# vision-agh/apse_uav

Measured on AMD Instinct MI355X. Metric: 4K UAV frames/sec (whole node), higher is better.
Workload: dtype f32

## Files before the change

### apse_uav_amd/_lib.py

```python
import ctypes as C
import os

import numpy as np

_HERE = os.path.dirname(os.path.abspath(__file__))
_TREE_LIB = os.path.join(_HERE, "libapse_hip.so")
LIB_PATH = os.environ.get("APSE_HIP_LIB") or _TREE_LIB
TOOL_ENTRIES = ("apse_conv2d_ex", "apse_winograd_pack_filter", "apse_winograd_conv2d", "apse_winograd_conv2d_split", "apse_conv_pointwise_launches", "apse_lane_stats", "apse_rpn_select", "apse_box_inference",
                "apse_c4_rpn_select", "apse_rpn_select_train", "apse_rpn_train_proposals_workspace_bytes", "apse_rpn_train_proposals",
                "apse_set_rpn_head", "apse_roi_features_windows", "apse_set_crop_features", "apse_preprocess_frames_yuv", "apse_yuv_to_bgr", "apse_yuv_matrix_host", "apse_resize_normalize_yuv")

APSE_OK = 0


class ApseError(RuntimeError):
    pass


class Config(C.Structure):
    _fields_ = [
        ("struct_size", C.c_int), ("device", C.c_int), ("max_batch", C.c_int),
        ("frame_h", C.c_int), ("frame_w", C.c_int), ("image_h", C.c_int), ("image_w", C.c_int),
        ("blocks", C.c_int * 4), ("num_classes", C.c_int),
        ("score_thresh", C.c_float), ("box_nms", C.c_float), ("rpn_nms", C.c_float), ("mask_thresh", C.c_float),
        ("rpn_pre_topk", C.c_int), ("rpn_post_topk", C.c_int), ("dets_per_image", C.c_int),
        ("pixel_mean", C.c_float * 3), ("assoc_roi", C.c_int), ("embed_dim", C.c_int), ("assoc_scale", C.c_float),
        ("compute_dtype", C.c_int), ("storage16", C.c_int),
    ]


class ConfigArch(Config):
    _fields_ = [("arch", C.c_int)]


class ConfigLane(ConfigArch):
    _fields_ = [("tail_lane", C.c_int)]


class ResultsLayout(C.Structure):
    _fields_ = [("bytes", C.c_size_t), ("n_max", C.c_int), ("dets_per_image", C.c_int), ("embed_dim", C.c_int),
                ("max_batch", C.c_int)] + [(k, C.c_size_t) for k in (
                    "total", "offset", "prop_count", "img", "cls", "roi", "score", "box_resized", "box", "valid", "rect",
                    "mass", "centroid", "closest", "embedding")]


class RenderItem(C.Structure):
    _fields_ = [("image", C.c_int), ("rect", C.c_int * 4), ("words_per_row", C.c_int), ("bits", C.c_void_p),
                ("box", C.c_float * 4), ("rgb", C.c_uint8 * 4), ("label_off", C.c_int), ("label_len", C.c_int)]


class MotsWindow(C.Structure):
    _fields_ = [("rect", C.c_int * 4), ("words_per_row", C.c_int), ("area", C.c_int), ("bits", C.c_void_p)]


class MotsObject(C.Structure):
    _fields_ = [("rect", C.c_int * 4), ("words_per_row", C.c_int), ("score", C.c_float), ("bits", C.c_void_p)]


class ConvDesc(C.Structure):
    _fields_ = [(k, C.c_int) for k in ("B", "H", "W", "Cin", "Cout", "KH", "KW", "stride", "pad", "relu", "res_mode",
                                       "cfg", "splitk", "prec", "fuse_reduce", "x_st", "res_st", "y_st")]


vp, i, f, sz = C.c_void_p, C.c_int, C.c_float, C.c_size_t
SIGNATURES = {
    "apse_create": ([C.POINTER(Config), C.POINTER(vp)], i),
    "apse_destroy": ([vp], None),
    "apse_last_error": ([vp], C.c_char_p),
    "apse_version": ([], C.c_char_p),
    "apse_set_weight": ([vp, C.c_char_p, vp, C.POINTER(C.c_int64), i], i),
    "apse_finalize_weights": ([vp], i),
    "apse_set_resize_tables": ([vp, vp, vp, i, vp, vp, i], i),
    "apse_set_camera": ([vp, C.POINTER(C.c_double), C.POINTER(C.c_double), i, vp, i, i], i),
    "apse_preprocess_frames": ([vp, vp, i, vp], i),
    "apse_preprocess_images": ([vp, vp, i, vp], i),
    "apse_backbone": ([vp, i, vp], i),
    "apse_rpn": ([vp, i, vp], i),
    "apse_rpn_levels": ([vp, i, i, vp], i),
    "apse_box_head": ([vp, i, vp], i),
    "apse_set_detections": ([vp, vp, vp, vp, vp, i, vp], i),
    "apse_mask_tail": ([vp, i, vp], i),
    "apse_embed": ([vp, i, vp], i),
    "apse_forward": ([vp, i, vp], i),
    "apse_results_describe": ([vp, C.POINTER(ResultsLayout)], i),
    "apse_read_results": ([vp, vp, sz, vp], i),
    "apse_read_results_begin": ([vp, vp, sz, vp], i),
    "apse_read_results_end": ([vp, vp], i),
    "apse_lane_stats": ([vp, C.POINTER(C.c_longlong * 4)], i),
    "apse_copy_mask_window": ([vp, i, i, i, i, i, vp, vp], i),
    "apse_copy_mask_windows": ([vp, i, vp, vp, vp, vp, vp], i),
    "apse_host_copy": ([vp, vp, sz, i], i),
    "apse_feature_shape": ([vp, C.c_char_p, C.POINTER(C.c_int * 3)], i),
    "apse_export_feature": ([vp, C.c_char_p, vp, i, vp], i),
    "apse_debug_tensor": ([vp, C.c_char_p, vp, sz, C.POINTER(sz), vp], i),
    "apse_flops": ([vp, i, C.c_double, C.c_double], C.c_double),
    "apse_profile": ([vp, i], i),
    "apse_profile_read": ([vp, C.POINTER(C.c_double * 42), i], i),
    "apse_conv_packed_elems": ([C.POINTER(ConvDesc)], sz),
    "apse_conv_pack_weight": ([C.POINTER(ConvDesc), vp, i, vp, vp], i),
    "apse_conv2d": ([C.POINTER(ConvDesc), vp, vp, vp, vp, vp, vp, sz, vp], i),
    "apse_conv2d_ex": ([C.POINTER(ConvDesc), vp, vp, vp, vp, vp, vp, sz, vp, i, i, i, vp], i),
    "apse_winograd_pack_filter": ([vp, i, i, vp], i),
    "apse_winograd_conv2d": ([C.POINTER(ConvDesc), vp, vp, vp, vp, vp], i),
    "apse_winograd_conv2d_split": ([C.POINTER(ConvDesc), vp, vp, vp, vp, vp, C.c_size_t, i, vp], i),
    "apse_conv_pointwise_launches": ([], C.c_uint),
    "apse_maxpool3x3s2": ([vp, vp, i, i, i, i, vp], i),
    "apse_maxpool3x3s2_typed": ([vp, vp, i, i, i, i, i, vp], i),
    "apse_roi_align": ([C.POINTER(vp), C.POINTER(i), C.POINTER(i), vp, i, i, i, vp, vp], i),
    "apse_roi_align_typed": ([C.POINTER(vp), C.POINTER(i), C.POINTER(i), vp, i, i, i, i, vp, vp], i),
    "apse_roi_pool": ([vp, i, i, vp, vp, i, i, f, vp, vp], i),
    "apse_roi_features": ([vp, i, vp, vp, i, i, vp, vp], i),
    "apse_roi_features_windows": ([vp, i, vp, vp, i, i, vp, vp], i),
    "apse_set_crop_features": ([vp, i], i),
    "apse_nms_rank": ([vp, vp, vp, i, i, i, i, f, i, vp, vp, vp, vp, vp], i),
    "apse_rpn_select": ([C.POINTER(vp), C.POINTER(i), C.POINTER(i), i, i, i, i, i, i, f, i, vp, vp, vp, vp, vp, vp, vp, vp, vp], i),
    "apse_box_inference": ([vp, i, i, vp, vp, i, i, i, i, f, f, i, i] + [vp] * 16, i),
    "apse_c4_rpn_select": ([vp, i, i, i, i, i, i, i, f, vp, vp, vp, vp, vp, vp, vp, vp], i),
    "apse_mask_centroid_dense": ([vp, i, i, C.POINTER(C.c_int * 3), vp], i),
    "apse_mask_closest_dense": ([vp, i, i, f, f, C.POINTER(C.c_int * 2), vp], i),
    "apse_l2_normalize": ([vp, vp, i, i, vp], i),
    "apse_sqdist": ([vp, vp, i, i, i, vp, vp], i),
    "apse_undistort_gamma": ([vp, vp, i, i, i, C.POINTER(C.c_double), C.POINTER(C.c_double), i, vp, i, i, vp], i),
    "apse_lab_tables_host": ([vp, vp, C.c_size_t], C.c_size_t),
    "apse_replay_create": ([i, i, f, i], vp),
    "apse_replay_destroy": ([vp], None),
    "apse_replay_step": ([vp, i, i, vp, vp, vp, C.c_char_p, i, vp], i),
    "apse_replay_packed": ([vp, vp, C.c_longlong, i, i, i, vp, C.c_longlong], C.c_longlong),
    "apse_replay_max_id": ([vp], i),
    "apse_replay_next_id": ([vp], i),
    "apse_render_workspace_bytes": ([i, i, i], sz),
    "apse_render_instances": ([vp, vp, i, i, i, i, vp, i, vp, sz, vp, i, vp, sz, vp], i),
    "apse_render_pack_mask": ([vp, i, i, vp, vp], i),
    "apse_render_font_host": ([vp, sz], sz),
    "apse_mots_split_workspace_bytes": ([], sz),
    "apse_mots_split_idmap": ([vp, i, i, i, vp, sz, vp, vp, vp, vp, sz, vp], i),
    "apse_mots_rle_to_bits": ([vp, vp, i, i, i, vp, vp], i),
    "apse_mots_overlaps": ([vp, i, vp, i, vp, i, vp, vp], i),
    "apse_mots_shift_overlaps": ([vp, i, vp, i, i, i, vp, vp], i),
    "apse_mots_render_idmap": ([vp, vp, i, i, i, vp, vp], i),
    "apse_mots_crop_overlaps": ([vp, vp, i, i, i, vp, sz, vp, vp, vp], i),
    "apse_mots_rle_workspace_bytes": ([vp, i, i, i], sz),
    "apse_mots_bits_to_rle": ([vp, vp, i, i, i, vp, i, vp, vp, vp, sz, vp], i),
    "apse_mots_rle_pack_workspace_bytes": ([i], sz),
    "apse_mots_rle_pack": ([vp, vp, i, i, vp, i, vp, vp, vp, sz, vp], i),
    "apse_resize_normalize": ([vp, vp, vp, vp, vp, vp, i, vp, vp, i, i, i, i, i, i, i, i, C.POINTER(f * 3), vp], i),
    "apse_assoc_fc_workspace_bytes": ([i, i, i], sz),
    "apse_assoc_fc_forward": ([vp, vp, vp, i, i, i, vp, vp, vp, sz, vp], i),
    "apse_assoc_fc_backward": ([vp, vp, vp, vp, i, i, i, vp, vp, vp, sz, vp], i),
    "apse_triplet_workspace_bytes": ([i], sz),
    "apse_triplet_hard_forward": ([vp, vp, i, i, f, i, vp, vp, sz, vp], i),
    "apse_triplet_all_forward": ([vp, vp, i, i, f, i, vp, vp, sz, vp], i),
    "apse_triplet_hard_backward": ([vp, i, i, i, vp, vp, vp, vp], i),
    "apse_triplet_all_backward": ([vp, i, i, i, vp, vp, vp, vp], i),
    "apse_sgd_step": ([vp, vp, vp, C.c_longlong, f, f, f, f, i, i, vp], i),
    "apse_coco_box_iou": ([vp, vp, vp, i, i, i, vp, vp, vp, vp, vp], i),
    "apse_coco_poly_to_bits": ([vp, vp, i, vp, i, vp, vp, vp, i, vp, vp, vp, vp], i),
    "apse_coco_match": ([vp, vp, vp, i, i, i, vp, vp, vp, i, vp, vp, vp, i, vp, i, vp, i, vp, vp, vp, vp, vp], i),
    "apse_coco_accumulate_workspace_bytes": ([C.c_longlong], sz),
# ... 90 lines not shown
```

### apse_uav_amd/csrc/conv_igemm.hip

```cpp
#include "apse_common.h"
#include <atomic>
#include <type_traits>

typedef _Float16 f16x8 __attribute__((ext_vector_type(8)));
__device__ __forceinline__ f32x16 apse_mfma16(bf16x8 a, bf16x8 b, f32x16 c) { return __builtin_amdgcn_mfma_f32_32x32x16_bf16(a, b, c, 0, 0, 0); }
__device__ __forceinline__ f32x16 apse_mfma16(f16x8 a, f16x8 b, f32x16 c) { return __builtin_amdgcn_mfma_f32_32x32x16_f16(a, b, c, 0, 0, 0); }

struct apse_pointwise {};
template <int WM, int WN, int TM, int TN, int KS, int XT, int WK, int PR = 0, typename... FORM>
__global__ __launch_bounds__(64 * WM * WN * WK) void conv_igemm_f32(const ConvParams p) {
    static_assert(sizeof...(FORM) == 0 || (sizeof...(FORM) == 1 && (std::is_same<FORM, apse_pointwise>::value && ...)), "FORM is nothing or apse_pointwise");
    constexpr bool PW = sizeof...(FORM) != 0;
    static_assert(PR == 0 || XT == 0, "16-bit operands use the descriptor path only");
    static_assert(!PW || XT == 0, "the pointwise address form exists for the plain descriptor path only");
    constexpr bool DESC = XT != 1;
    constexpr int EPS = PR ? 64 : 32;
    constexpr int ESH = PR ? 1 : 2;
    constexpr int EPSLOT = 16 >> ESH;
    constexpr int NT = 64 * WM * WN * WK;
    constexpr int BM = WM * TM * 32;
    constexpr int BN = WN * TN * 32;
    constexpr int SR = NT / 8;
    constexpr int AP = BM / SR;
    constexpr int BP = BN / SR;
    static_assert(AP >= 1 && BP >= 1 && KS % WK == 0 && (DESC || WK == 1), "unsupported shape");
    constexpr int LDC = BN + 4;
    constexpr bool DP = DESC && (TM * TN <= 2 || (PR != 0 && WM * WN == 8 && APSE_DP16));
    constexpr int NSET = DP ? 2 : 1;
    constexpr int STORE_AT = 4 * KS - 2;
    extern __shared__ __attribute__((aligned(16))) char smem[];
    float* As = reinterpret_cast<float*>(smem);
    float* Bs = As + 2 * KS * BM * 32;
    float* Cs = reinterpret_cast<float*>(smem);

    const int tid = threadIdx.x;
    const int lane = tid & 63;
    const int wave = tid >> 6;
    const int kg = wave / (WM * WN);
    const int wm = (wave % (WM * WN)) / WN, wn = wave % WN;
    const int fr = lane & 31, fh = lane >> 5;
    const int srow = tid >> 3, slot = tid & 7;

    int M = p.M;
    if (p.m_count) {
        int lim = (*p.m_count) * p.m_per_item;
        M = lim < M ? lim : M;
    }
    const int tiles_n = (p.Cout + BN - 1) / BN;
    const int tiles_m = (M + BM - 1) / BM;
    const int nwg = tiles_m * tiles_n;
    const int z = blockIdx.y;
    const int steps_per_row = p.KWCp / EPS;
    const int steps_total = PR ? p.KH * steps_per_row : p.steps_total;
    const int steps_big = (steps_total + KS - 1) / KS;
    const int per = (steps_big + p.splitk - 1) / p.splitk;
    const int s_begin = z * per;
    const int s_end = (s_begin + per < steps_big) ? s_begin + per : steps_big;
    const int ohw = p.OH * p.OW;
    const size_t w_row = (size_t)p.KH * p.KWCp;
    const bool direct = (p.splitk == 1);
    __amdgpu_buffer_rsrc_t xrsrc;
    const unsigned xbytes = (((unsigned)(p.B * p.H * p.W) << p.cin_log2)) << (XT >= 2 ? 1 : ESH);
    if constexpr (DESC)
        xrsrc = __builtin_amdgcn_make_buffer_rsrc(const_cast<float*>(p.x), 0, (int)xbytes, 0x00020000);
    __amdgpu_buffer_rsrc_t wrsrc;
    if constexpr (PW)
        wrsrc = __builtin_amdgcn_make_buffer_rsrc(PR ? const_cast<void*>(reinterpret_cast<const void*>(p.w16)) : const_cast<void*>(reinterpret_cast<const void*>(p.w)), 0,
                                                  (int)(((unsigned)((p.Cout + 127) & ~127) * (unsigned)w_row) << ESH), 0x00020000);

    bool warm_pending = p.next_w && z == 0;
    for (int wg = blockIdx.x; wg < nwg; wg += gridDim.x) {
        const int bid = apse_xcd_remap(wg, nwg);
        const int tile_m = bid / tiles_n, tile_n = bid - tile_m * tiles_n;
        const int m0 = tile_m * BM, n0 = tile_n * BN;

        int a_iy0[AP], a_ix0[AP], a_pix[AP], a_base[AP];
#pragma unroll
        for (int i = 0; i < AP; ++i) {
            const int m = m0 + srow + SR * i;
            if (m < M) {
                const int b = m / ohw;
                const int rem = m - b * ohw;
                const int oy = rem / p.OW;
                const int ox = rem - oy * p.OW;
                a_iy0[i] = oy * p.stride - p.pad;
                a_ix0[i] = ox * p.stride - p.pad;
                a_pix[i] = b * p.H * p.W;
            } else {
                a_iy0[i] = -(1 << 28);
                a_ix0[i] = 0;
                a_pix[i] = 0;
            }
            a_base[i] = (a_pix[i] + a_iy0[i] * p.W + a_ix0[i]) << p.cin_log2;
        }

        f32x4 ra[NSET][KS][AP], rb[NSET][KS][BP];
        int ld_r, ld_q;
        {
            const int ss0 = s_begin * KS;
            ld_r = ss0 / steps_per_row;
            ld_q = ss0 - ld_r * steps_per_row;
        }
        const char* wrow[BP];
#pragma unroll
        for (int i = 0; i < BP; ++i)
            wrow[i] = (PR ? reinterpret_cast<const char*>(p.w16) : reinterpret_cast<const char*>(p.w)) +
                      ((((size_t)(n0 + srow + SR * i) * w_row) + (size_t)(slot * EPSLOT)) << ESH);
        int cur_r = 0, cur_ry = 0, cur_q = 0, cur_rowoff = 0, cur_woff = 0, cur_dpx = 0;
        unsigned pw_a[AP], pw_w[BP];
        int pw_s = s_begin * KS, pw_soff = 0;
        unsigned pw_xbytes = 0;
        if constexpr (PW) {
#pragma unroll
            for (int i = 0; i < AP; ++i) {
                const bool in = ((unsigned)a_iy0[i] < (unsigned)p.H) & ((unsigned)a_ix0[i] < (unsigned)p.W);
                pw_a[i] = in ? ((unsigned)(a_base[i] + slot * EPSLOT) << ESH) : 0xfffffff0u;
            }
#pragma unroll
            for (int i = 0; i < BP; ++i) pw_w[i] = ((unsigned)(n0 + srow + SR * i) * (unsigned)w_row + (unsigned)(slot * EPSLOT)) << ESH;
        }
        auto fetch_piece = [&](int set, int u, int j) {
            if constexpr (PW) {
                if (j == 0) {
                    const bool live = pw_s < steps_total;
                    pw_soff = live ? pw_s * 128 : 0;
                    pw_xbytes = live ? xbytes : 0u;
                    ++pw_s;
                }
                if (j < AP) {
                    const __amdgpu_buffer_rsrc_t xs = __builtin_amdgcn_make_buffer_rsrc(const_cast<float*>(p.x), 0, (int)pw_xbytes, 0x00020000);
                    ra[set][u][j] = __builtin_bit_cast(f32x4, __builtin_amdgcn_raw_buffer_load_b128(xs, (int)pw_a[j], pw_soff, 0));
                } else {
                    rb[set][u][j - AP] = __builtin_bit_cast(f32x4, __builtin_amdgcn_raw_buffer_load_b128(wrsrc, (int)pw_w[j - AP], pw_soff, 0));
                }
                return;
            }
            if (j == 0) {
                const bool live = ld_r < p.KH;
                cur_r = live ? ld_r : p.KH - 1;
                cur_ry = live ? ld_r : (1 << 28);
                cur_q = ld_q * EPS + slot * EPSLOT;
                cur_dpx = cur_q >> p.cin_log2;
                cur_rowoff = ((cur_r * p.W) << p.cin_log2) + cur_q;
                cur_woff = (cur_r * p.KWCp + ld_q * EPS) << ESH;
                ++ld_q;
                if (ld_q == steps_per_row) { ld_q = 0; ++ld_r; }
            }
            if (j < AP) {
                const int iy = a_iy0[j] + cur_ry;
                const int px = a_ix0[j] + cur_dpx;
                const int okm = -(int)(((unsigned)iy < (unsigned)p.H) & ((unsigned)px < (unsigned)p.W));
                if constexpr (XT >= 2) {
                    const unsigned off = (((unsigned)(a_base[j] + cur_rowoff) << 1) & (unsigned)okm) | (0xfffffff0u & ~(unsigned)okm);
                    const auto raw = __builtin_amdgcn_raw_buffer_load_b64(xrsrc, (int)off, 0, 0);
                    ra[set][u][j] = f32x4{__uint_as_float(raw[0]), __uint_as_float(raw[1]), 0.f, 0.f};
                } else {
                    const unsigned off = (((unsigned)(a_base[j] + cur_rowoff) << ESH) & (unsigned)okm) | (0xfffffff0u & ~(unsigned)okm);
                    ra[set][u][j] = __builtin_bit_cast(f32x4, __builtin_amdgcn_raw_buffer_load_b128(xrsrc, (int)off, 0, 0));
                }
            } else {
                rb[set][u][j - AP] = *reinterpret_cast<const f32x4*>(wrow[j - AP] + cur_woff);
            }
        };
        auto store_piece = [&](int set, int buf, int u, int j) {
            if (j < AP) {
                const int row = srow + SR * j;
                const int ps = slot ^ ((row >> 1) & 7);
                f32x4 v = ra[set][u][j];
                if constexpr (XT == 2) {
                    const unsigned lo = __float_as_uint(v[0]), hi = __float_as_uint(v[1]);
                    v = f32x4{__uint_as_float(lo << 16), __uint_as_float(lo & 0xffff0000u), __uint_as_float(hi << 16), __uint_as_float(hi & 0xffff0000u)};
                } else if constexpr (XT == 3) {
                    typedef _Float16 h2 __attribute__((ext_vector_type(2)));
                    const h2 a = __builtin_bit_cast(h2, __float_as_uint(v[0])), b = __builtin_bit_cast(h2, __float_as_uint(v[1]));
                    v = f32x4{(float)a[0], (float)a[1], (float)b[0], (float)b[1]};
                }
                *reinterpret_cast<f32x4*>(As + (buf * KS + u) * BM * 32 + row * 32 + ps * 4) = v;
            } else {
                const int row = srow + SR * (j - AP);
                const int ps = slot ^ ((row >> 1) & 7);
                *reinterpret_cast<f32x4*>(Bs + (buf * KS + u) * BN * 32 + row * 32 + ps * 4) = rb[set][u][j - AP];
            }
        };
        auto load_step_bl = [&](int set) {
#pragma unroll
            for (int u = 0; u < KS; ++u)
// ... 437 lines not shown
__global__ __launch_bounds__(256) void conv_splitk_reduce(const ConvParams p) {
    int M = p.M;
    if (p.m_count) {
        int lim = (*p.m_count) * p.m_per_item;
        M = lim < M ? lim : M;
    }
    const size_t total = (size_t)M * p.Cout;
    const int ohw = p.OH * p.OW;
    for (size_t e = (size_t)blockIdx.x * blockDim.x + threadIdx.x; e < total; e += (size_t)gridDim.x * blockDim.x) {
        const int m = (int)(e / p.Cout);
        const int n = (int)(e - (size_t)m * p.Cout);
        float val = 0.f;
        for (int z = 0; z < p.splitk; ++z) val += p.ws[((size_t)z * p.M + m) * p.Cout + n];
        int co = n, g = 0;
        if (p.out_mode == 1) { g = n / p.cdec; co = n - g * p.cdec; }
        if (p.bias) val += p.bias[co];
        auto ld1 = [&](size_t idx) -> float {
            if (p.res_st == 0) return p.res[idx];
            if (p.res_st == 1) return __uint_as_float((uint32_t)reinterpret_cast<const uint16_t*>(p.res)[idx] << 16);
            return (float)reinterpret_cast<const _Float16*>(p.res)[idx];
        };
        size_t dst;
        if (p.out_mode == 0) {
            if (p.res_mode == 1) {
                val += ld1((size_t)m * p.Cout + n);
            } else if (p.res_mode == 2) {
                const int b = m / ohw;
                const int rem = m - b * ohw;
                const int oy = rem / p.OW, ox = rem - oy * p.OW;
                const int hw2 = (p.OH >> 1) * (p.OW >> 1);
                val += ld1(((size_t)b * hw2 + (oy >> 1) * (p.OW >> 1) + (ox >> 1)) * p.Cout + n);
            }
            dst = (size_t)m * p.y_ld + p.y_coff + n;
        } else {
            const int b = m / ohw;
            const int rem = m - b * ohw;
            const int oy = rem / p.OW, ox = rem - oy * p.OW;
            const int dy = g >> 1, dx = g & 1;
            dst = (((size_t)b * 2 * p.OH + 2 * oy + dy) * (2 * p.OW) + 2 * ox + dx) * p.cdec + co;
        }
        if (p.relu) val = apse_relu(val);
        apse_st1(p.y, dst, val, p.y_st);
    }
}

void apse_launch_splitk_reduce4(const ConvParams& p, hipStream_t s) {
    int blocks = (int)(((size_t)p.M * p.Cout / 4 + 255) / 256);
    if (blocks > 4096) blocks = 4096;
    hipLaunchKernelGGL(conv_splitk_reduce4, dim3(blocks), dim3(256), 0, s, p);
}

static std::atomic<unsigned> g_pointwise_launches{0};
extern "C" unsigned apse_conv_pointwise_launches(void) { return g_pointwise_launches.load(std::memory_order_relaxed); }

template <int WM, int WN, int TM, int TN, int KS, int XT, int WK = 1, int PR = 0, bool PW = false>
static int launch_cfg_x(const ConvParams& p, hipStream_t s, hipEvent_t ev0, hipEvent_t ev1) {
    constexpr int BM = WM * TM * 32, BN = WN * TN * 32;
    const int tiles = ((p.M + BM - 1) / BM) * ((p.Cout + BN - 1) / BN);
    const size_t lds_stage = (size_t)2 * KS * (BM + BN) * 32 * sizeof(float), lds_c = (size_t)WK * BM * (BN + 4) * sizeof(float) + 16;
    const size_t lds = lds_stage > lds_c ? lds_stage : lds_c;
    static bool attr_done = false;
    if (!attr_done) {
        if constexpr (PW)
            hipFuncSetAttribute(reinterpret_cast<const void*>(&conv_igemm_f32<WM, WN, TM, TN, KS, XT, WK, PR, apse_pointwise>),
                                hipFuncAttributeMaxDynamicSharedMemorySize, (int)lds);
        else
            hipFuncSetAttribute(reinterpret_cast<const void*>(&conv_igemm_f32<WM, WN, TM, TN, KS, XT, WK, PR>),
                                hipFuncAttributeMaxDynamicSharedMemorySize, (int)lds);
        attr_done = true;
    }
    int grid_x = tiles;
    if (p.m_count) {
        int want = 1024;
        if (p.m_hint > 0) {
            want = 2 * ((p.m_hint + BM - 1) / BM) * ((p.Cout + BN - 1) / BN);
            if (want < 64) want = 64;
            if (want > 1024) want = 1024;
        }
        if (grid_x > want) grid_x = want;
    }
    if (ev0) hipEventRecord(ev0, s);
    if constexpr (PW) {
        hipLaunchKernelGGL((conv_igemm_f32<WM, WN, TM, TN, KS, XT, WK, PR, apse_pointwise>), dim3(grid_x, p.splitk), dim3(64 * WM * WN * WK), lds, s, p);
        g_pointwise_launches.fetch_add(1, std::memory_order_relaxed);
    } else {
        hipLaunchKernelGGL((conv_igemm_f32<WM, WN, TM, TN, KS, XT, WK, PR>), dim3(grid_x, p.splitk), dim3(64 * WM * WN * WK), lds, s, p);
    }
    if (ev1) hipEventRecord(ev1, s);
    if (p.splitk > 1 && !p.tile_cnt) {
        const size_t total = (size_t)p.M * p.Cout;
        const bool vec4 = p.out_mode == 0 && (p.res_mode == 0 || p.res_mode == 1) && ((p.Cout | p.y_ld | p.y_coff) & 3) == 0 && total < 0x7fffffffull;
        int blocks = (int)(((vec4 ? total / 4 : total) + 255) / 256);
        if (blocks > 4096) blocks = 4096;
        if (vec4) hipLaunchKernelGGL(conv_splitk_reduce4, dim3(blocks), dim3(256), 0, s, p);
        else hipLaunchKernelGGL(conv_splitk_reduce, dim3(blocks), dim3(256), 0, s, p);
    }
    return hipGetLastError() == hipSuccess ? APSE_OK : APSE_E_HIP;
}

static bool descriptor_ok(const ConvParams& p) { return p.x_st == 0 && (((size_t)p.B * p.H * p.W) << p.cin_log2) * 4 < 0xfffffff0ull; }

static bool igemm_addr_on() {
    static const bool on = [] { const char* e = getenv("APSE_IGEMM_ADDR"); return !(e && e[0] == '0'); }();
    return on;
}
static bool pointwise_ok(const ConvParams& p) {
    return igemm_addr_on() && p.KH == 1 && p.KW == 1 && p.pad == 0 && p.KWCp == (1 << p.cin_log2) &&
           (size_t)((p.Cout + 127) & ~127) * (size_t)p.KWCp * 4 < 0xfffffff0ull;
}

template <int WM, int WN, int TM, int TN, int KS, bool PWF = false>
static int launch_cfg(const ConvParams& p, hipStream_t s, hipEvent_t ev0, hipEvent_t ev1) {
    if (!descriptor_ok(p)) return launch_cfg_x<WM, WN, TM, TN, KS, 1>(p, s, ev0, ev1);
    if constexpr (PWF)
        if (pointwise_ok(p)) return launch_cfg_x<WM, WN, TM, TN, KS, 0, 1, 0, true>(p, s, ev0, ev1);
    return launch_cfg_x<WM, WN, TM, TN, KS, 0>(p, s, ev0, ev1);
}
template <int WM, int WN, int TM, int TN, int KS, int KSF, bool PWF = false>
static int launch_cfg_k2(const ConvParams& p, hipStream_t s, hipEvent_t ev0, hipEvent_t ev1) {
    if (!descriptor_ok(p)) return launch_cfg_x<WM, WN, TM, TN, KSF, 1>(p, s, ev0, ev1);
    if constexpr (PWF)
        if (pointwise_ok(p)) return launch_cfg_x<WM, WN, TM, TN, KS, 0, 2, 0, true>(p, s, ev0, ev1);
    return launch_cfg_x<WM, WN, TM, TN, KS, 0, 2>(p, s, ev0, ev1);
}
template <int WM, int WN, int TM, int TN, int KS, int WK, int PR>
static int launch_cfg16(const ConvParams& p, hipStream_t s, hipEvent_t ev0, hipEvent_t ev1) {
    if (pointwise_ok(p)) return launch_cfg_x<WM, WN, TM, TN, KS, 0, WK, PR, true>(p, s, ev0, ev1);
    return launch_cfg_x<WM, WN, TM, TN, KS, 0, WK, PR>(p, s, ev0, ev1);
}

static int fast16_shape(const ConvParams& p, int cfg) {
    const bool fast16 = (p.prec == 1 || p.prec == 2) && p.w16 && p.x_st == p.prec && (p.KWCp & 63) == 0 && p.cin_log2 >= 3 &&
                        ((((size_t)p.B * p.H * p.W) << p.cin_log2) * 2 < 0xfffffff0ull) && !p.tile_cnt;
    if (!fast16) return -1;
    int c16 = (cfg == 4 || cfg == 5 || cfg == 2) ? 1 : (cfg == 7 ? 6 : cfg);
    if (c16 == 0 && p.steps_total >= 16 && ((p.M + 255) / 256) * ((p.Cout + 127) / 128) >= 250) c16 = 8;
    return c16;
}

int apse_conv_effective_cfg(const ConvParams& p, int cfg) {
    if (cfg == APSE_CFG_STREAM) return (!p.no_stream && apse_conv1x1_stream_ok(p)) ? APSE_CFG_STREAM : -1;
    if (cfg == APSE_CFG_GLDS) return apse_conv_glds16_ok(p) ? APSE_CFG_GLDS : -1;
    if (cfg == APSE_CFG_SKINNY) return apse_conv_skinny_ok(p) ? APSE_CFG_SKINNY : -1;
    if (!p.no_stream && apse_conv_skinny_ok(p)) return APSE_CFG_SKINNY;
    if (!p.no_stream && apse_conv1x1_stream_ok(p)) return APSE_CFG_STREAM;
    if (!p.no_stream && apse_conv_glds16_ok(p)) {
        const int c16 = fast16_shape(p, cfg);
        if (c16 == 8) return APSE_CFG_GLDS;
        const int t128 = ((p.M + 127) / 128) * ((p.Cout + 127) / 128);
        if ((c16 == 0 || c16 == 3) && p.steps_total >= 16 && t128 >= 200 && t128 <= 320 && apse_conv_glds16_small(p)) return APSE_CFG_GLDS;
    }
    return cfg;
}

int apse_launch_conv(const ConvParams& p, int cfg, hipStream_t s, hipEvent_t ev0, hipEvent_t ev1) {
    if (p.M <= 0 || p.Cout <= 0 || p.steps_total <= 0) return APSE_E_INVALID;
    if (p.res_mode != 0 && (p.Cout & 3) != 0) return APSE_E_INVALID;
    const int eff = apse_conv_effective_cfg(p, cfg);
    if (eff < 0) return APSE_E_INVALID;
    if (eff == APSE_CFG_STREAM) return apse_launch_conv1x1_stream(p, s, ev0, ev1);
    if (eff == APSE_CFG_GLDS) return apse_launch_conv_glds16(p, s, ev0, ev1);
    if (eff == APSE_CFG_SKINNY) return apse_launch_conv_skinny(p, s, ev0, ev1);
    if (p.prec == 1 || p.prec == 2) {
        const int c16 = fast16_shape(p, cfg);
        if (c16 >= 0) {
            int rc = APSE_E_INVALID;
            if (p.prec == 1) {
                if (c16 == 0) rc = launch_cfg16<2, 2, 2, 2, 1, 1, 1>(p, s, ev0, ev1);
                else if (c16 == 1) rc = launch_cfg16<2, 2, 1, 1, 2, 1, 1>(p, s, ev0, ev1);
                else if (c16 == 3) rc = launch_cfg16<4, 1, 1, 2, 1, 1, 1>(p, s, ev0, ev1);
                else if (c16 == 6) rc = launch_cfg16<2, 2, 1, 1, 2, 2, 1>(p, s, ev0, ev1);
                else if (c16 == 8) rc = launch_cfg_x<4, 2, 2, 2, 1, 0, 1, 1>(p, s, ev0, ev1);
            } else {
                if (c16 == 0) rc = launch_cfg16<2, 2, 2, 2, 1, 1, 2>(p, s, ev0, ev1);
                else if (c16 == 1) rc = launch_cfg16<2, 2, 1, 1, 2, 1, 2>(p, s, ev0, ev1);
                else if (c16 == 3) rc = launch_cfg16<4, 1, 1, 2, 1, 1, 2>(p, s, ev0, ev1);
                else if (c16 == 6) rc = launch_cfg16<2, 2, 1, 1, 2, 2, 2>(p, s, ev0, ev1);
                else if (c16 == 8) rc = launch_cfg_x<4, 2, 2, 2, 1, 0, 1, 2>(p, s, ev0, ev1);
            }
            return rc;
        }
        return APSE_E_INVALID;
    }
    switch (cfg) {
        case 0: return launch_cfg<2, 2, 2, 2, 1, true>(p, s, ev0, ev1);
        case 1: return launch_cfg<2, 2, 1, 1, 2, true>(p, s, ev0, ev1);
        case 2: {
            const bool small = (((size_t)p.B * p.H * p.W) << p.cin_log2) * 4 < 0xfffffff0ull;
            if (small && p.x_st == 1 && p.cin_log2 >= 2) return launch_cfg_x<4, 1, 1, 1, 2, 2>(p, s, ev0, ev1);
            if (small && p.x_st == 2 && p.cin_log2 >= 2) return launch_cfg_x<4, 1, 1, 1, 2, 3>(p, s, ev0, ev1);
            return launch_cfg<4, 1, 1, 1, 2>(p, s, ev0, ev1);
        }
        case 3: return launch_cfg<4, 1, 1, 2, 1, true>(p, s, ev0, ev1);
        case 4: return launch_cfg<2, 2, 1, 1, 1>(p, s, ev0, ev1);
        case 5: return launch_cfg<4, 1, 1, 1, 1>(p, s, ev0, ev1);
        case 6: return launch_cfg_k2<2, 2, 1, 1, 2, 2, true>(p, s, ev0, ev1);
        case 7: return launch_cfg_k2<2, 2, 1, 1, 4, 2>(p, s, ev0, ev1);
        case 8: return launch_cfg<2, 2, 2, 2, 1>(p, s, ev0, ev1);
        default: return APSE_E_INVALID;
    }
}

int apse_conv_pick_cfg(int M, int Cout, int steps, int* splitk) {
    *splitk = 1;
    auto tiles = [&](int bm, int bn) { return ((M + bm - 1) / bm) * ((Cout + bn - 1) / bn); };
    auto split_for = [&](int t, int min_steps_per_split) {
        int sk = (512 + t / 2) / t;
        if (sk > steps / min_steps_per_split) sk = steps / min_steps_per_split;
        if (sk > 64) sk = 64;
        return sk < 1 ? 1 : sk;
    };
    if (Cout <= 32) {
        const int t = tiles(128, 32);
        if (t < 32 && steps >= 16) {
            int sk = 64 / t;
            if (sk > steps / 4) sk = steps / 4;
            if (sk > 8) sk = 8;
            *splitk = sk < 1 ? 1 : sk;
        }
        return 2;
    }
    if (Cout <= 64) return tiles(128, 64) >= 192 ? 3 : 1;
    const int t128 = tiles(128, 128);
    if (t128 >= 224) {
        if (t128 < 384 && tiles(128, 64) >= 384) return 3;
        return 0;
    }
    if (t128 >= 32 && steps >= 256) {
        *splitk = split_for(t128, 8);
        return 0;
    }
    const int t64 = tiles(64, 64);
    if (t64 >= 192) return t64 <= 320 ? 6 : 1;
    if (steps >= 16) {
        int sk = (256 + t64 / 2) / t64;
        if (t64 > 64 && sk > 2) sk = 2;
        if (sk > steps / 8) sk = steps / 8;
        if (sk > 64) sk = 64;
        *splitk = sk < 1 ? 1 : sk;
        return 6;
    }
    return 1;
}
```

### include/apse_hip.h

```cpp
#ifndef APSE_HIP_H
#define APSE_HIP_H
#include <stddef.h>
#include <stdint.h>
#ifdef __cplusplus
extern "C" {
#endif

#define APSE_OK 0
#define APSE_E_INVALID (-1)
#define APSE_E_HIP (-2)
#define APSE_E_NOMEM (-3)
#define APSE_E_STATE (-4)
#define APSE_E_MISSING (-5)

typedef struct apse_ctx apse_ctx;

#define APSE_MAX_CLASSES 80
#define APSE_C4_MAX_PRE_TOPK 6000
#define APSE_C4_MAX_BATCH 2
#define APSE_MAX_FRAME_W 49152
#define APSE_MAX_FRAME_H 32768
typedef struct apse_config {
    int struct_size;
    int device;
// ... 57 lines not shown
int apse_preprocess_frames_yuv(apse_ctx* ctx, const uint8_t* frames_dev, int batch, int pitch, int format, int matrix, void* stream);
int apse_preprocess_images(apse_ctx* ctx, const float* images_dev, int batch, void* stream);
int apse_backbone(apse_ctx* ctx, int batch, void* stream);
int apse_rpn(apse_ctx* ctx, int batch, void* stream);
int apse_rpn_levels(apse_ctx* ctx, int batch, int level_mask, void* stream);
int apse_box_head(apse_ctx* ctx, int batch, void* stream);
int apse_set_detections(apse_ctx* ctx, const float* boxes_host, const int* classes_host, const float* scores_host,
                        const int* counts_host, int batch, void* stream);
int apse_mask_tail(apse_ctx* ctx, int batch, void* stream);
int apse_embed(apse_ctx* ctx, int batch, void* stream);
int apse_roi_features(apse_ctx* ctx, int image, const float* rois_dev, const uint8_t* masks_dev, int n, int roi_size,
                      float* out_dev, void* stream);
struct apse_mots_window;
int apse_roi_features_windows(apse_ctx* ctx, int image, const float* rois_dev, const struct apse_mots_window* windows_dev, int n,
                              int roi_size, float* out_dev, void* stream);
int apse_set_crop_features(apse_ctx* ctx, int on);
int apse_forward(apse_ctx* ctx, int batch, void* stream);

int apse_results_describe(apse_ctx* ctx, apse_results_layout* out);
int apse_read_results(apse_ctx* ctx, void* host_dst, size_t bytes, void* stream);
int apse_read_results_begin(apse_ctx* ctx, void* host_dst, size_t bytes, void* stream);
int apse_read_results_end(apse_ctx* ctx, void* host_dst);
int apse_lane_stats(apse_ctx* ctx, long long* out4);
int apse_copy_mask_window(apse_ctx* ctx, int det, int x0, int y0, int x1, int y1, uint64_t* dst_dev, void* stream);
int apse_copy_mask_windows(apse_ctx* ctx, int n, const int* dets_host, const int* rects_host, uint64_t* dst_dev,
                           const long long* dst_word_offsets_host, void* stream);
int apse_feature_shape(apse_ctx* ctx, const char* name, int* chw3);
int apse_export_feature(apse_ctx* ctx, const char* name, float* dst_nchw_dev, int batch, void* stream);
int apse_debug_tensor(apse_ctx* ctx, const char* name, void* dst_dev, size_t max_bytes, size_t* bytes, void* stream);
double apse_flops(apse_ctx* ctx, int batch, double proposals, double detections);

int apse_profile(apse_ctx* ctx, int enable);
int apse_profile_read(apse_ctx* ctx, double* out42, int reset);

typedef struct apse_conv_desc {
    int B, H, W, Cin;
    int Cout, KH, KW, stride, pad;
    int relu;
    int res_mode;
    int cfg;
    int splitk;
    int prec;
    int fuse_reduce;
    int x_st, res_st, y_st;
} apse_conv_desc;
size_t apse_conv_packed_elems(const apse_conv_desc* d);
int apse_conv_pack_weight(const apse_conv_desc* d, const float* w_oihw, int cin_real, const float* scale, float* packed);
int apse_conv2d(const apse_conv_desc* d, const float* x_dev, const float* w_packed_dev, const float* bias_dev,
                const float* res_dev, float* y_dev, float* ws_dev, size_t ws_bytes, void* stream);
int apse_conv2d_ex(const apse_conv_desc* d, const void* x_dev, const float* w_packed_dev, const float* bias_dev, const void* res_dev,
                   void* y_dev, float* ws_dev, size_t ws_bytes, const int* count_dev, int hint_items, int y_ld, int deconv,
                   void* stream);
unsigned apse_conv_pointwise_launches(void);
int apse_winograd_pack_filter(const float* w_oihw, int Cout, int Cin, float* packed);
int apse_winograd_conv2d(const apse_conv_desc* d, const float* x_dev, const float* wu_dev, const float* bias_dev, float* y_dev,
                         void* stream);
int apse_winograd_conv2d_split(const apse_conv_desc* d, const float* x_dev, const float* wu_dev, const float* bias_dev, float* y_dev,
                               float* ws_dev, size_t ws_bytes, int geometry, void* stream);
int apse_maxpool3x3s2(const float* x_dev, float* y_dev, int B, int H, int W, int C, void* stream);
int apse_maxpool3x3s2_typed(const void* x_dev, void* y_dev, int B, int H, int W, int C, int storage, void* stream);
int apse_roi_align(const float* const* feats_dev, const int* hs, const int* ws, const float* rois_dev, int n, int per_img,
                   int out_size, float* out_dev, void* stream);
int apse_roi_align_typed(const void* const* feats_dev, const int* hs, const int* ws, const float* rois_dev, int n, int per_img,
                         int out_size, int storage, void* out_dev, void* stream);
int apse_roi_pool(const float* feat_dev, int H, int W, const float* rois_dev, const int* roi_img_dev, int n, int out_size,
                  float scale, float* out_dev, void* stream);
int apse_nms_rank(const float* boxes_dev, const float* scores_dev, const int* valid_dev, int n, int cat_div, int cat_mod,
                  int ncat, float thr, int topk, float* out_boxes_dev, float* out_scores_dev, int* out_index_dev,
                  int* out_count_dev, void* stream);
int apse_rpn_select(const float* const* heads_dev, const int* H, const int* W, int head_ld, int B, int image_h, int image_w,
                    int pre_topk, int post_topk, float nms_thr, int level_mask, unsigned long long* keys_dev, float* dec_boxes_dev,
                    float* dec_scores_dev, int* dec_valid_dev, float* props_dev, float* prop_scores_dev, int* prop_entry_dev,
                    int* prop_count_dev, void* stream);
int apse_box_inference(const float* pred_dev, int ld, int K, const float* props_dev, const int* prop_cnt_dev, int P, int B,
                       int image_h, int image_w, float score_thresh, float nms_thr, int dets_per_image, int wide,
                       float* probs_dev, float* cand_boxes_dev, float* cand_scores_dev, int* cand_valid_dev, float* det_boxes_dev,
                       float* det_scores_dev, int* det_entry_dev, int* det_cnt_dev, float* pk_boxes_dev, float* pk_scores_dev,
                       int* pk_cls_dev, int* pk_img_dev, int* pk_roi_dev, int* pk_total_dev, int* pk_offset_dev, void* stream);
int apse_c4_rpn_select(const float* head_dev, int H, int W, int B, int image_h, int image_w, int pre, int post, float nms_thr,
                       float* dec_boxes_dev, float* dec_scores_dev, int* dec_valid_dev, float* props_dev, float* prop_scores_dev,
                       int* prop_entry_dev, int* prop_count_dev, void* stream);
int apse_mask_centroid_dense(const uint8_t* mask_dev, int H, int W, int* out_xy_mass_host3, void* stream);
int apse_mask_closest_dense(const uint8_t* mask_dev, int H, int W, float px, float py, int* out_xy_host2, void* stream);
int apse_l2_normalize(const float* x_dev, float* y_dev, int n, int D, void* stream);
int apse_sqdist(const float* a_dev, const float* b_dev, int O, int N, int D, float* out_dev, void* stream);
int apse_undistort_gamma(const uint8_t* src_dev, uint8_t* dst_dev, int B, int H, int W, const double* mtx3x3_host,
                         const double* dist_host, int ndist, const uint8_t* lut256_host, int do_undistort, int do_gamma,
                         void* stream);
size_t apse_lab_tables_host(const uint8_t* lut256_host, void* out, size_t cap);
int apse_resize_normalize(const uint8_t* frames_dev, uint8_t* tmp_dev, float* out_nhwc4_dev, uint8_t* resized_u8_dev,
                          const int* hb_dev, const int* hc_dev, int hk, const int* vb_dev, const int* vc_dev, int vk, int B,
                          int H, int W, int OH, int OW, int PH, int PW, const float* mean3_host, void* stream);

#define APSE_FMT_NV12 0
#define APSE_FMT_I420 1
#define APSE_YUV_CV601 0
#define APSE_YUV_BT601 1
#define APSE_YUV_BT709 2
#define APSE_YUV_BT601_FULL 3
#define APSE_YUV_BT709_FULL 4
int apse_yuv_to_bgr(const uint8_t* src_dev, uint8_t* dst_dev, int B, int H, int W, int pitch, int format, int matrix, void* stream);
int apse_yuv_matrix_host(int matrix, int* out6);
int apse_resize_normalize_yuv(const uint8_t* frames_dev, int pitch, int format, int matrix, uint8_t* tmp_dev, float* out_nhwc4_dev,
                              uint8_t* resized_u8_dev, const int* hb_dev, const int* hc_dev, int hk, const int* vb_dev,
                              const int* vc_dev, int vk, int B, int H, int W, int OH, int OW, int PH, int PW,
                              const float* mean3_host, void* stream);
// ... 204 lines not shown
```

Baseline: 208.8.

## Add tap-wise incremental addressing path for KxK implicit-GEMM convolutions

Adds an 'apse_taps' address form to the f32 implicit-GEMM conv kernel for spatial (KxK) convolutions with power-of-two channel counts. Instead of recomputing per-step input coordinates and bounds checks, it precomputes a per-row padding bitmask and base offsets once per tile, then advances scalar offsets per tap, wrapping at each kernel row. Out-of-image taps are zeroed through buffer-load range checks against a shifted base pointer. The goal is to cut the address arithmetic in the load loop, at the cost of more kernel instantiations and subtle offset/mask logic. It is enabled by default for cfg 1 and 6, with an env override to disable it.

```diff
diff --git a/apse_uav_amd/_lib.py b/apse_uav_amd/_lib.py
--- a/apse_uav_amd/_lib.py
+++ b/apse_uav_amd/_lib.py
@@ -6,7 +6,7 @@
 _HERE = os.path.dirname(os.path.abspath(__file__))
 _TREE_LIB = os.path.join(_HERE, "libapse_hip.so")
 LIB_PATH = os.environ.get("APSE_HIP_LIB") or _TREE_LIB
-TOOL_ENTRIES = ("apse_conv2d_ex", "apse_winograd_pack_filter", "apse_winograd_conv2d", "apse_winograd_conv2d_split", "apse_conv_pointwise_launches", "apse_lane_stats", "apse_rpn_select", "apse_box_inference",
+TOOL_ENTRIES = ("apse_conv2d_ex", "apse_winograd_pack_filter", "apse_winograd_conv2d", "apse_winograd_conv2d_split", "apse_conv_pointwise_launches", "apse_conv_taps_launches", "apse_lane_stats", "apse_rpn_select", "apse_box_inference",
                 "apse_c4_rpn_select", "apse_rpn_select_train", "apse_rpn_train_proposals_workspace_bytes", "apse_rpn_train_proposals",
                 "apse_set_rpn_head", "apse_roi_features_windows", "apse_set_crop_features", "apse_preprocess_frames_yuv", "apse_yuv_to_bgr", "apse_yuv_matrix_host", "apse_resize_normalize_yuv")
 
@@ -104,6 +104,7 @@
     "apse_winograd_conv2d": ([C.POINTER(ConvDesc), vp, vp, vp, vp, vp], i),
     "apse_winograd_conv2d_split": ([C.POINTER(ConvDesc), vp, vp, vp, vp, vp, C.c_size_t, i, vp], i),
     "apse_conv_pointwise_launches": ([], C.c_uint),
+    "apse_conv_taps_launches": ([], C.c_uint),
     "apse_maxpool3x3s2": ([vp, vp, i, i, i, i, vp], i),
     "apse_maxpool3x3s2_typed": ([vp, vp, i, i, i, i, i, vp], i),
     "apse_roi_align": ([C.POINTER(vp), C.POINTER(i), C.POINTER(i), vp, i, i, i, vp, vp], i),
diff --git a/apse_uav_amd/csrc/conv_igemm.hip b/apse_uav_amd/csrc/conv_igemm.hip
--- a/apse_uav_amd/csrc/conv_igemm.hip
+++ b/apse_uav_amd/csrc/conv_igemm.hip
@@ -7,10 +7,17 @@
 __device__ __forceinline__ f32x16 apse_mfma16(f16x8 a, f16x8 b, f32x16 c) { return __builtin_amdgcn_mfma_f32_32x32x16_f16(a, b, c, 0, 0, 0); }
 
 struct apse_pointwise {};
+struct apse_taps {};
+struct apse_taps1 {};
 template <int WM, int WN, int TM, int TN, int KS, int XT, int WK, int PR = 0, typename... FORM>
 __global__ __launch_bounds__(64 * WM * WN * WK) void conv_igemm_f32(const ConvParams p) {
-    static_assert(sizeof...(FORM) == 0 || (sizeof...(FORM) == 1 && (std::is_same<FORM, apse_pointwise>::value && ...)), "FORM is nothing or apse_pointwise");
-    constexpr bool PW = sizeof...(FORM) != 0;
+    static_assert(sizeof...(FORM) == 0 || (sizeof...(FORM) == 1 && ((std::is_same<FORM, apse_pointwise>::value || std::is_same<FORM, apse_taps>::value || std::is_same<FORM, apse_taps1>::value) && ...)),
+                  "FORM is nothing, apse_pointwise, apse_taps or apse_taps1");
+    constexpr bool PW = (std::is_same<FORM, apse_pointwise>::value || ...);
+    constexpr bool TP1 = (std::is_same<FORM, apse_taps1>::value || ...);
+    constexpr bool TP = TP1 || (std::is_same<FORM, apse_taps>::value || ...);
+    constexpr int TPW = TP1 ? 1 : 2;
+    static_assert(!TP || (XT == 0 && PR == 0 && KS == 2), "the taps address form exists for the plain f32 descriptor path at 64-deep steps only");
     static_assert(PR == 0 || XT == 0, "16-bit operands use the descriptor path only");
     static_assert(!PW || XT == 0, "the pointwise address form exists for the plain descriptor path only");
     constexpr bool DESC = XT != 1;
@@ -64,9 +71,14 @@
     if constexpr (DESC)
         xrsrc = __builtin_amdgcn_make_buffer_rsrc(const_cast<float*>(p.x), 0, (int)xbytes, 0x00020000);
     __amdgpu_buffer_rsrc_t wrsrc;
-    if constexpr (PW)
+    if constexpr (PW || TP)
         wrsrc = __builtin_amdgcn_make_buffer_rsrc(PR ? const_cast<void*>(reinterpret_cast<const void*>(p.w16)) : const_cast<void*>(reinterpret_cast<const void*>(p.w)), 0,
                                                   (int)(((unsigned)((p.Cout + 127) & ~127) * (unsigned)w_row) << ESH), 0x00020000);
+    const unsigned tp_back = (((unsigned)(p.pad * p.W + p.pad)) << p.cin_log2) << 2;
+    const char* const tp_x = reinterpret_cast<const char*>(p.x) - tp_back;
+    const int tp_sh = p.cin_log2 + 2;
+    const int tp_wrap = ((p.W - p.KW) << p.cin_log2) << 2;
+    const int tp_bend = steps_total * 128;
 
     bool warm_pending = p.next_w && z == 0;
     for (int wg = blockIdx.x; wg < nwg; wg += gridDim.x) {
@@ -110,6 +122,28 @@
         unsigned pw_a[AP], pw_w[BP];
         int pw_s = s_begin * KS, pw_soff = 0;
         unsigned pw_xbytes = 0;
+        unsigned tp_a[AP], tp_m[AP];
+        int tp_b = 0, tp_rq = 0, tp_row = 0;
+        int tp_sa = 0, tp_sb = 0, tp_t = 0;
+        unsigned tp_xb = 0;
+        if constexpr (TP) {
+            const unsigned kw_all = 0xffffffffu >> (32 - p.KW);
+#pragma unroll
+            for (int i = 0; i < AP; ++i) {
+                unsigned cols = 0, msk = 0;
+                for (int dx = 0; dx < p.KW; ++dx) cols |= ((unsigned)(a_ix0[i] + dx) < (unsigned)p.W ? 0u : 1u) << dx;
+                for (int r = p.KH - 1; r >= 0; --r) msk = (msk << p.KW) | ((unsigned)(a_iy0[i] + r) < (unsigned)p.H ? cols : kw_all);
+                tp_m[i] = msk;
+                tp_a[i] = ((unsigned)(a_base[i] + slot * EPSLOT) << ESH) + tp_back;
+            }
+#pragma unroll
+            for (int i = 0; i < BP; ++i) pw_w[i] = ((unsigned)(n0 + srow + SR * i) * (unsigned)w_row + (unsigned)(slot * EPSLOT)) << ESH;
+            const int ss0 = s_begin * KS;
+            const int r0 = ss0 / steps_per_row;
+            tp_rq = ss0 - r0 * steps_per_row;
+            tp_row = r0 * tp_wrap;
+            tp_b = ss0 * 128;
+        }
         if constexpr (PW) {
 #pragma unroll
             for (int i = 0; i < AP; ++i) {
@@ -132,6 +166,28 @@
                     ra[set][u][j] = __builtin_bit_cast(f32x4, __builtin_amdgcn_raw_buffer_load_b128(xs, (int)pw_a[j], pw_soff, 0));
                 } else {
                     rb[set][u][j - AP] = __builtin_bit_cast(f32x4, __builtin_amdgcn_raw_buffer_load_b128(wrsrc, (int)pw_w[j - AP], pw_soff, 0));
+                }
+                return;
+            }
+            if constexpr (TP) {
+                if (j == 0 && u % TPW == 0) {
+                    tp_sb = tp_b < tp_bend - 128 * TPW ? tp_b : tp_bend - 128 * TPW;
+                    tp_xb = tp_b < tp_bend ? xbytes + tp_back : 0u;
+                    tp_sa = tp_b + tp_row;
+                    tp_t = tp_b >> tp_sh;
+                    tp_b += 128 * TPW;
+                    tp_rq += TPW;
+                    if (tp_rq == steps_per_row) { tp_rq = 0; tp_row += tp_wrap; }
+                } else if (j == 0) {
+                    tp_sa += 128;
+                    tp_sb += 128;
+                }
+                if (j < AP) {
+                    const __amdgpu_buffer_rsrc_t xs = __builtin_amdgcn_make_buffer_rsrc(const_cast<char*>(tp_x), 0, (int)tp_xb, 0x00020000);
+                    const unsigned off = tp_a[j] | (unsigned)__builtin_amdgcn_sbfe((int)tp_m[j], (unsigned)tp_t, 1u);
+                    ra[set][u][j] = __builtin_bit_cast(f32x4, __builtin_amdgcn_raw_buffer_load_b128(xs, (int)off, tp_sa, 0));
+                } else {
+                    rb[set][u][j - AP] = __builtin_bit_cast(f32x4, __builtin_amdgcn_raw_buffer_load_b128(wrsrc, (int)pw_w[j - AP], tp_sb, 0));
                 }
                 return;
             }
@@ -675,8 +731,10 @@
 
 static std::atomic<unsigned> g_pointwise_launches{0};
 extern "C" unsigned apse_conv_pointwise_launches(void) { return g_pointwise_launches.load(std::memory_order_relaxed); }
-
-template <int WM, int WN, int TM, int TN, int KS, int XT, int WK = 1, int PR = 0, bool PW = false>
+static std::atomic<unsigned> g_taps_launches{0};
+extern "C" unsigned apse_conv_taps_launches(void) { return g_taps_launches.load(std::memory_order_relaxed); }
+
+template <int WM, int WN, int TM, int TN, int KS, int XT, int WK = 1, int PR = 0, bool PW = false, int TP = 0>
 static int launch_cfg_x(const ConvParams& p, hipStream_t s, hipEvent_t ev0, hipEvent_t ev1) {
     constexpr int BM = WM * TM * 32, BN = WN * TN * 32;
     const int tiles = ((p.M + BM - 1) / BM) * ((p.Cout + BN - 1) / BN);
@@ -687,6 +745,12 @@
         if constexpr (PW)
             hipFuncSetAttribute(reinterpret_cast<const void*>(&conv_igemm_f32<WM, WN, TM, TN, KS, XT, WK, PR, apse_pointwise>),
                                 hipFuncAttributeMaxDynamicSharedMemorySize, (int)lds);
+        else if constexpr (TP == 2)
+            hipFuncSetAttribute(reinterpret_cast<const void*>(&conv_igemm_f32<WM, WN, TM, TN, KS, XT, WK, PR, apse_taps>),
+                                hipFuncAttributeMaxDynamicSharedMemorySize, (int)lds);
+        else if constexpr (TP == 1)
+            hipFuncSetAttribute(reinterpret_cast<const void*>(&conv_igemm_f32<WM, WN, TM, TN, KS, XT, WK, PR, apse_taps1>),
+                                hipFuncAttributeMaxDynamicSharedMemorySize, (int)lds);
         else
             hipFuncSetAttribute(reinterpret_cast<const void*>(&conv_igemm_f32<WM, WN, TM, TN, KS, XT, WK, PR>),
                                 hipFuncAttributeMaxDynamicSharedMemorySize, (int)lds);
@@ -706,6 +770,12 @@
     if constexpr (PW) {
         hipLaunchKernelGGL((conv_igemm_f32<WM, WN, TM, TN, KS, XT, WK, PR, apse_pointwise>), dim3(grid_x, p.splitk), dim3(64 * WM * WN * WK), lds, s, p);
         g_pointwise_launches.fetch_add(1, std::memory_order_relaxed);
+    } else if constexpr (TP == 2) {
+        hipLaunchKernelGGL((conv_igemm_f32<WM, WN, TM, TN, KS, XT, WK, PR, apse_taps>), dim3(grid_x, p.splitk), dim3(64 * WM * WN * WK), lds, s, p);
+        g_taps_launches.fetch_add(1, std::memory_order_relaxed);
+    } else if constexpr (TP == 1) {
+        hipLaunchKernelGGL((conv_igemm_f32<WM, WN, TM, TN, KS, XT, WK, PR, apse_taps1>), dim3(grid_x, p.splitk), dim3(64 * WM * WN * WK), lds, s, p);
+        g_taps_launches.fetch_add(1, std::memory_order_relaxed);
     } else {
         hipLaunchKernelGGL((conv_igemm_f32<WM, WN, TM, TN, KS, XT, WK, PR>), dim3(grid_x, p.splitk), dim3(64 * WM * WN * WK), lds, s, p);
     }
@@ -723,27 +793,44 @@
 
 static bool descriptor_ok(const ConvParams& p) { return p.x_st == 0 && (((size_t)p.B * p.H * p.W) << p.cin_log2) * 4 < 0xfffffff0ull; }
 
-static bool igemm_addr_on() {
-    static const bool on = [] { const char* e = getenv("APSE_IGEMM_ADDR"); return !(e && e[0] == '0'); }();
-    return on;
-}
+static int igemm_addr_mode() {
+    static const int mode = [] {
+        const char* e = getenv("APSE_IGEMM_ADDR");
+        if (e && e[0] == '0') return 0;
+        return (e && e[0] == 'p' && e[1] == 'w' && e[2] == 0) ? 1 : 2;
+    }();
+    return mode;
+}
+static bool igemm_addr_on() { return igemm_addr_mode() != 0; }
 static bool pointwise_ok(const ConvParams& p) {
     return igemm_addr_on() && p.KH == 1 && p.KW == 1 && p.pad == 0 && p.KWCp == (1 << p.cin_log2) &&
            (size_t)((p.Cout + 127) & ~127) * (size_t)p.KWCp * 4 < 0xfffffff0ull;
 }
 
-template <int WM, int WN, int TM, int TN, int KS, bool PWF = false>
+static bool taps_ok(const ConvParams& p) {
+    return igemm_addr_mode() == 2 && !pointwise_ok(p) && p.cin_log2 >= 5 && p.KWCp == (p.KW << p.cin_log2) && p.KH * p.KW <= 32 && p.pad >= 0 &&
+           (size_t)((p.Cout + 127) & ~127) * (size_t)p.KH * (size_t)p.KWCp * 4 < 0xfffffff0ull &&
+           ((((size_t)p.B * p.H * p.W) + (size_t)p.pad * p.W + p.pad) << p.cin_log2) * 4 < 0xfffffff0ull;
+}
+
+template <int WM, int WN, int TM, int TN, int KS, bool PWF = false, bool TPF = false>
 static int launch_cfg(const ConvParams& p, hipStream_t s, hipEvent_t ev0, hipEvent_t ev1) {
     if (!descriptor_ok(p)) return launch_cfg_x<WM, WN, TM, TN, KS, 1>(p, s, ev0, ev1);
     if constexpr (PWF)
         if (pointwise_ok(p)) return launch_cfg_x<WM, WN, TM, TN, KS, 0, 1, 0, true>(p, s, ev0, ev1);
+    if constexpr (TPF)
+        if (taps_ok(p))
+            return p.cin_log2 >= 6 ? launch_cfg_x<WM, WN, TM, TN, KS, 0, 1, 0, false, 2>(p, s, ev0, ev1) : launch_cfg_x<WM, WN, TM, TN, KS, 0, 1, 0, false, 1>(p, s, ev0, ev1);
     return launch_cfg_x<WM, WN, TM, TN, KS, 0>(p, s, ev0, ev1);
 }
-template <int WM, int WN, int TM, int TN, int KS, int KSF, bool PWF = false>
+template <int WM, int WN, int TM, int TN, int KS, int KSF, bool PWF = false, bool TPF = false>
 static int launch_cfg_k2(const ConvParams& p, hipStream_t s, hipEvent_t ev0, hipEvent_t ev1) {
     if (!descriptor_ok(p)) return launch_cfg_x<WM, WN, TM, TN, KSF, 1>(p, s, ev0, ev1);
     if constexpr (PWF)
         if (pointwise_ok(p)) return launch_cfg_x<WM, WN, TM, TN, KS, 0, 2, 0, true>(p, s, ev0, ev1);
+    if constexpr (TPF)
+        if (taps_ok(p))
+            return p.cin_log2 >= 6 ? launch_cfg_x<WM, WN, TM, TN, KS, 0, 2, 0, false, 2>(p, s, ev0, ev1) : launch_cfg_x<WM, WN, TM, TN, KS, 0, 2, 0, false, 1>(p, s, ev0, ev1);
     return launch_cfg_x<WM, WN, TM, TN, KS, 0, 2>(p, s, ev0, ev1);
 }
 template <int WM, int WN, int TM, int TN, int KS, int WK, int PR>
@@ -807,7 +894,7 @@
     }
     switch (cfg) {
         case 0: return launch_cfg<2, 2, 2, 2, 1, true>(p, s, ev0, ev1);
-        case 1: return launch_cfg<2, 2, 1, 1, 2, true>(p, s, ev0, ev1);
+        case 1: return launch_cfg<2, 2, 1, 1, 2, true, true>(p, s, ev0, ev1);
         case 2: {
             const bool small = (((size_t)p.B * p.H * p.W) << p.cin_log2) * 4 < 0xfffffff0ull;
             if (small && p.x_st == 1 && p.cin_log2 >= 2) return launch_cfg_x<4, 1, 1, 1, 2, 2>(p, s, ev0, ev1);
@@ -817,7 +904,7 @@
         case 3: return launch_cfg<4, 1, 1, 2, 1, true>(p, s, ev0, ev1);
         case 4: return launch_cfg<2, 2, 1, 1, 1>(p, s, ev0, ev1);
         case 5: return launch_cfg<4, 1, 1, 1, 1>(p, s, ev0, ev1);
-        case 6: return launch_cfg_k2<2, 2, 1, 1, 2, 2, true>(p, s, ev0, ev1);
+        case 6: return launch_cfg_k2<2, 2, 1, 1, 2, 2, true, true>(p, s, ev0, ev1);
         case 7: return launch_cfg_k2<2, 2, 1, 1, 4, 2>(p, s, ev0, ev1);
         case 8: return launch_cfg<2, 2, 2, 2, 1>(p, s, ev0, ev1);
         default: return APSE_E_INVALID;
diff --git a/include/apse_hip.h b/include/apse_hip.h
--- a/include/apse_hip.h
+++ b/include/apse_hip.h
@@ -133,6 +133,7 @@
                    void* y_dev, float* ws_dev, size_t ws_bytes, const int* count_dev, int hint_items, int y_ld, int deconv,
                    void* stream);
 unsigned apse_conv_pointwise_launches(void);
+unsigned apse_conv_taps_launches(void);
 int apse_winograd_pack_filter(const float* w_oihw, int Cout, int Cin, float* packed);
 int apse_winograd_conv2d(const apse_conv_desc* d, const float* x_dev, const float* wu_dev, const float* bias_dev, float* y_dev,
                          void* stream);
```

New measurement: 212.8 (median of 6 runs). Within noise of the previous version (+1.9%).
